# shichaoy/pop_up_slam

Hardware: AMD Instinct MI355X
Metric: graph-solve iters/sec + final chi2, 1k-pose/5k-edge plane graph (higher is better)
Workload: dtype f64; 1 GPU; C2 synthetic corridor: 1000 SE3 poses, 200 planes, 5000 plane edges, 999 odometry edges (BASELINE.json configs[1], seed 42); jacobian_mode=numeric, total_lm_solves=805

## Files before the change

pop_up_slam_amd/csrc/pps_api.cpp:

```cpp
#include "pps_graph.h"

using namespace pps;
using namespace pps_impl;

namespace pps {
Switches read_switches() {
  auto on = [](const char* k) { return getenv(k) != nullptr; };
  auto num = [](const char* k, long long dflt) { const char* e = getenv(k); return e && *e ? atoll(e) : dflt; };
  Switches s;
  s.k1_thread_form = on("PPS_K1_THREAD_FORM");
  {
    long long plain = num("PPS_PLAIN_SCHEDULE", 0);
    if (on("PPS_PLAIN_SCHEDULE") && plain <= 0) plain = 15;
    s.no_preassemble = (plain & 1) != 0; s.no_solve_flow = (plain & 2) != 0; s.no_root_fuse = (plain & 4) != 0; s.split_expand = (plain & 8) != 0;
  }
  s.no_spec_lin = on("PPS_NO_SPEC_LIN");
  s.no_dual = on("PPS_NO_DUAL");
  s.no_strip = on("PPS_NO_STRIP");
  s.no_incremental = on("PPS_NO_INCREMENTAL");
  s.no_incr_compact = on("PPS_NO_INCR_COMPACT");
  s.verify_upload = on("PPS_DEBUG_VERIFY_UPLOAD");
  s.multi_levels = on("PPS_MULTI_LEVELS");
  s.multi_thread_form = on("PPS_MULTI_THREAD_FORM");
  s.debug_drop_flag = (int)num("PPS_DEBUG_DROP_FLAG", 0);
  if (on("PPS_DEBUG_DROP_FLAG") && s.debug_drop_flag < 1) s.debug_drop_flag = 1;
  s.trace = (int)num("PPS_TRACE", 0);
  if (on("PPS_TRACE") && s.trace < 1) s.trace = 1;
  {
    long long tm = num("PPS_TIMING", 0);
    if (on("PPS_TIMING") && tm <= 0) tm = 7;
    s.analysis_timing = (tm & 1) != 0; s.upload_timing = (tm & 2) != 0; s.multi_timing = (tm & 8) ? 2 : ((tm & 4) ? 1 : 0);
  }
  s.multi_split = (int)num("PPS_MULTI_SPLIT", 0);
  s.multi_thread_factors = num("PPS_MULTI_THREAD_FACTORS", 120000);
  return s;
}
}

namespace pps_impl {
void report_front_trace(pps_graph* g) {
  const Analysis& A = g->an;
  std::vector<long long> tr((size_t)A.n_fronts * 8);
  (void)hipMemcpy(tr.data(), g->dev.trace, tr.size() * 8, hipMemcpyDeviceToHost);
  if (g->dev.trace_solve) {
    for (int l = A.n_levels - 1; l >= 0; l--) {
      double ph[5] = {0, 0, 0, 0, 0}, gap = 0; int n = 0, ng = 0;
      for (int s2 = 0; s2 < A.n_fronts; s2++) {
        if (A.f_level[s2] != l) continue;
        n++;
        for (int k = 0; k < 5; k++) ph[k] += (double)(tr[(size_t)s2 * 8 + k + 1] - tr[(size_t)s2 * 8 + k]);
        const int par = A.f_parent[s2];
        if (par >= 0) { gap += (double)(tr[(size_t)s2 * 8] - tr[(size_t)par * 8 + 5]); ng++; }
      }
      if (!n) continue;
      fprintf(stderr, "  solve level %d (%d fronts): panel load %.0f boundary values %.0f y - L_B^T x_b %.0f back-substitution %.0f store %.0f | start after parent's end %.0f\n",
              l, n, ph[0] / n, ph[1] / n, ph[2] / n, ph[3] / n, ph[4] / n, ng ? gap / ng : 0.0);
    }
  } else {
    double acc[5] = {0, 0, 0, 0, 0};
    std::vector<double> lvl_tot(A.n_levels, 0.0); std::vector<int> lvl_n(A.n_levels, 0);
    for (int s2 = 0; s2 < A.n_fronts; s2++) {
      for (int k = 0; k < 5; k++) acc[k] += (double)(tr[(size_t)s2 * 8 + k + 1] - tr[(size_t)s2 * 8 + k]);
      lvl_tot[A.f_level[s2]] += (double)(tr[(size_t)s2 * 8 + 5] - tr[(size_t)s2 * 8]); lvl_n[A.f_level[s2]]++;
    }
    { double pn = 0, tr2 = 0; for (int s2 = 0; s2 < A.n_fronts; s2++) { pn += (double)tr[(size_t)s2 * 8 + 6]; tr2 += (double)tr[(size_t)s2 * 8 + 7]; }
      fprintf(stderr, "PPS_TRACE elimination split: panel %.0f trailing %.0f cycles per front\n", pn / A.n_fronts, tr2 / A.n_fronts); }
    fprintf(stderr, "PPS_TRACE mean cycles per front: zero %.0f gather %.0f extend-add %.0f eliminate %.0f store %.0f\n",
// ... 523 lines not shown
```

pop_up_slam_amd/csrc/pps_device.h:

```cpp
#pragma once

#include <hip/hip_runtime.h>

#include <cstdint>

namespace pps {

struct DevGraph {
  int n_pose = 0, n_plane = 0, pose_ld = 0, plane_ld = 0;
  double *pose_est = nullptr, *pose_lin = nullptr;
  double *plane_est = nullptr, *plane_lin = nullptr;
  int *pose_voff = nullptr, *plane_voff = nullptr;
  int n_obs = 0, n_odo = 0, n_pp = 0, n_lp = 0;
  int obs_ld = 0, odo_ld = 0, pp_ld = 0, lp_ld = 0;
  int *obs_pose = nullptr, *obs_plane = nullptr; double *obs_meas = nullptr, *obs_w = nullptr;
  int n_obs_fixed = 0; double* obs_ray = nullptr;
  int *odo_a = nullptr, *odo_b = nullptr;         double *odo_meas = nullptr, *odo_w = nullptr;
  int *pp_pose = nullptr;                          double *pp_meas = nullptr, *pp_w = nullptr;
  int *lp_plane = nullptr;                         double *lp_meas = nullptr, *lp_w = nullptr;
  double* J = nullptr;
  int64_t joff_obs = 0, joff_odo = 0, joff_pp = 0, joff_lp = 0;
  double* P = nullptr;
  int64_t poff_obs = 0;
  double* H = nullptr;
  double* L = nullptr;
  double* U = nullptr;
  double* delta = nullptr;
  int n_scalars = 0;
  int n_fronts = 0, n_levels = 0, max_front = 0, n_segs = 0, n_blocks = 0;
  int *f_p = nullptr, *f_b = nullptr, *f_poff = nullptr;
  int* pidx = nullptr;
  int64_t *f_Loff = nullptr, *f_Uoff = nullptr;
  int *f_bidx_off = nullptr, *bidx = nullptr;
  int *f_child_off = nullptr, *child = nullptr;
  int *f_cmap_off = nullptr, *cmap = nullptr;
  int *level_fronts = nullptr;
  int *f_asm_off = nullptr, *asm_blk = nullptr, *asm_lrow = nullptr, *asm_lcol = nullptr;
  int *asm_el0 = nullptr, *asm_fsz = nullptr;
  int *blk_rows = nullptr, *blk_cols = nullptr, *blk_size = nullptr, *blk_nseg = nullptr;
  int64_t* blk_hoff = nullptr;
  int *seg_blk = nullptr, *seg_c0 = nullptr, *seg_cnt = nullptr;
  int64_t* seg_hoff = nullptr;
  int* contrib = nullptr;
  int n_mseg = 0; int* mseg_blk = nullptr;
  int *f_el_off = nullptr, *el_src = nullptr, *el_tgt = nullptr;
  int *blk_doff = nullptr, *blk_dst = nullptr;
  double* Hf = nullptr;
  int64_t* f_ea_off = nullptr; int* ea_tgt = nullptr;
  int *grp_lvl_off = nullptr, *glvl_front_off = nullptr, *glvl_fronts = nullptr;
  int* grp_span = nullptr;
  int *frec = nullptr, *crec = nullptr, *srec = nullptr;
  int* obs_dir = nullptr;
  int* k3_flag = nullptr;
  int* nd_segs = nullptr; int n_nd_segs = 0;
  int* k2_single = nullptr; int n_k2_single = 0;
  int* k2_multi = nullptr; int n_k2_multi = 0;
  int* k2_finish = nullptr; int n_k2_finish = 0;
  int* k2t = nullptr; int n_k2t_big = 0, n_k2t_small = 0, n_k2t_spec = 0;
  int *cls_off = nullptr, *cls_fronts = nullptr;
  double* chi2_partials = nullptr;
  int chi2_blocks = 0;
  double* dn_partials = nullptr;
  unsigned int* ticket = nullptr;
  double* result_dev = nullptr;
  long long* trace = nullptr;
  int trace_solve = 0;
  int no_strip = 0;
  unsigned sw = 0;
  double step_ac[4] = {0, 0, 0, 0};
  double* gwork = nullptr;
  int64_t gwork_stride = 0;
};

constexpr double kStatusInternal = 64.0;
enum : unsigned { SW_K1_THREAD_FORM = 1u, SW_NO_SOLVE_FLOW = 2u, SW_NO_ROOT_FUSE = 4u, SW_DEBUG_DROP_FLAG = 8u, SW_DEBUG_DROP_XFLAG = 16u };
struct Switches {
  bool k1_thread_form = false;
  bool no_preassemble = false;
  bool no_solve_flow = false;
  bool no_root_fuse = false;
  bool split_expand = false;
  bool no_spec_lin = false;
  bool no_dual = false;
  bool no_strip = false;
  bool no_incremental = false;
  bool no_incr_compact = false;
  bool verify_upload = false;
  bool multi_levels = false, multi_thread_form = false;
  int debug_drop_flag = 0;
  int trace = 0;
  bool analysis_timing = false, upload_timing = false;
  int multi_timing = 0;
  int multi_split = 0;
  long long multi_thread_factors = 120000;
  unsigned dev_bits() const {
    return (k1_thread_form ? SW_K1_THREAD_FORM : 0u) | (no_solve_flow ? SW_NO_SOLVE_FLOW : 0u) | (no_root_fuse ? SW_NO_ROOT_FUSE : 0u) |
           (debug_drop_flag == 1 ? SW_DEBUG_DROP_FLAG : 0u) | (debug_drop_flag == 2 ? SW_DEBUG_DROP_XFLAG : 0u);
  }
};
Switches read_switches();

struct LinGuard {
  const double* chi[2];
  const double* pose[2];
  const double* plane[2];
  double error;
  int on, single;
  int want = -1;
};

struct SpecLin {
  double *J, *P, *H, *Hf;
  int which;
};

unsigned long long launch_count();
void count_launch();
#define PPS_LAUNCH(...) do { ::pps::count_launch(); hipLaunchKernelGGL(__VA_ARGS__); } while (0)
#define PPS_LAUNCH_EV(ev0, ev1, kernel, grid, block, lds, st, ...)                                                     \
  do {                                                                                                                 \
    ::pps::count_launch();                                                                                             \
    if (ev0) hipExtLaunchKernelGGL(kernel, grid, block, lds, st, ev0, ev1, 0, __VA_ARGS__);                            \
    else hipLaunchKernelGGL(kernel, grid, block, lds, st, __VA_ARGS__);                                                \
  } while (0)

hipError_t step_constants(double ac[4]);
hipError_t launch_linearize(const DevGraph& d, int mode, bool at_estimate, hipStream_t st, const LinGuard* guard = nullptr, hipEvent_t ev0 = nullptr,
                            hipEvent_t ev1 = nullptr);
hipError_t launch_hblocks(const DevGraph& d, hipStream_t st, const LinGuard* guard = nullptr, bool products = true);
bool k1_lane_form(const DevGraph& d, int mode);
bool k1_products(const DevGraph& d, int mode);
hipError_t launch_factor_level(const DevGraph& d, int level_begin, int level_count, int level_max_front, double lambda,
                               hipStream_t st);
hipError_t launch_backsolve_level(const DevGraph& d, int level_begin, int level_count, hipStream_t st);
struct DualAlt {
  double *L, *U, *delta, *result_dev, *chi2_partials, *dn_partials;
  unsigned int* ticket;
  double lambda;
};
hipError_t launch_band_all(const DevGraph& d, const DualAlt* alt, int n_groups, int nwaves_factor, int nwaves_solve, int max_front, int max_panel,
                           int max_group_fronts, double lambda, int epoch, hipStream_t st, hipEvent_t ev0 = nullptr, hipEvent_t ev1 = nullptr);
int band_all_solve_waves(int max_panel, int max_group_fronts);
hipError_t launch_band_factor(const DevGraph& d, int grp_begin, int grp_count, int nwaves, int max_front, double lambda, hipStream_t st,
                              hipEvent_t ev0 = nullptr, hipEvent_t ev1 = nullptr, bool pre = false);
hipError_t launch_band_solve(const DevGraph& d, int grp_begin, int grp_count, int nwaves, int max_panel, int max_group_fronts, hipStream_t st,
                             const DualAlt* alt = nullptr);
hipError_t launch_band_factor_dual(const DevGraph& d, const DualAlt& alt, int grp_begin, int grp_count, int nwaves, int max_front, double lambda,
                                   hipStream_t st, hipEvent_t ev0 = nullptr, hipEvent_t ev1 = nullptr, bool pre = false);
bool band_root_fusable(const DevGraph& d, int grp_count, int max_front);
hipError_t launch_band_root(const DevGraph& d, const DualAlt* alt, int grp, int nwaves_factor, int nwaves_solve, int max_front, int max_panel,
// ... 96 lines not shown
```

pop_up_slam_amd/csrc/pps_front_reg.h:

```cpp
#pragma once
#include <type_traits>

#include "pps_regtile.h"

namespace pps {

#ifndef PPS_TR
#define PPS_TR(k) do { if (d.trace && lane == 0) d.trace[(size_t)s * 8 + (k)] = clock64(); } while (0)
#endif

__device__ __forceinline__ int tri(int i) { return (i * (i + 1)) >> 1; }
__device__ __forceinline__ int tri24(int i) { return __mul24(i, i + 1) >> 1; }

template <int NT, bool TR, bool STRIP, int W = 8, class G>
__device__ __forceinline__ void front_reg_eliminate(const G& d, int rec, double* F, double* P) {
  const int lane = threadIdx.x & 63;
  const int s = __builtin_amdgcn_readlane(rec, 0), p = __builtin_amdgcn_readlane(rec, 1), b = __builtin_amdgcn_readlane(rec, 2);
  const int l16 = lane & 15, lq = lane >> 4;
  const int f = p + b, fa = f + 1;
  const bool strip = STRIP && fa > kRegRows;
  constexpr bool R5 = NT == 5;
  const int mr = STRIP ? fa : f;
  (void)s;
  double4_t c[NT * (NT + 1) / 2];
#pragma unroll
  for (int ti = 0; ti < NT; ti++)
#pragma unroll
    for (int r = 0; r < 4; r++) {
      const int row = 16 * ti + lq + 4 * r;
      const double* Fr = F + (tri24(row < mr ? row : 0) + l16);
#pragma unroll
      for (int tj = 0; tj <= ti; tj++) c[tile_id(ti, tj)][r] = Fr[16 * tj];
    }
  double y = 0.0;
  if (!STRIP) { const double t = F[lane <= f ? tri24(f) + lane : 0]; y = lane < f ? t : 0.0; }
  __builtin_amdgcn_wave_barrier();
  double* __restrict__ Lp = d.L + (((long long)__builtin_amdgcn_readlane(rec, 10) << 32) | (unsigned int)__builtin_amdgcn_readlane(rec, 9));
  long long cyc_panel = 0, cyc_trail = 0;
  bool bad = false;
  auto panel_step = [&](const int K) __attribute__((always_inline)) {
    const long long tk0 = (TR && d.trace) ? clock64() : 0;
    const int nb = p - K < W ? p - K : W;
    const bool two = nb > 4;
    const int tjK = K >> 4, c0 = K & 15;
    switch (tjK) {
      case 0: reg_extract_panel8<0, NT>(c, P, c0, lane); break;
      case 1: reg_extract_panel8<1, NT>(c, P, c0, lane); break;
      case 2: if (NT > 2) reg_extract_panel8<(NT > 2 ? 2 : 1), NT>(c, P, c0, lane); break;
      default: if (NT > 3) reg_extract_panel8<(NT > 3 ? 3 : NT - 1), NT>(c, P, c0, lane); break;
    }
    const int row2 = kRegRows + (lane & 15);
    const bool has2 = STRIP && strip && lane < 16 && row2 < fa;
    if (has2 && !R5) {
#pragma unroll
      for (int m = 0; m < 8; m++) P[row2 * kP8Stride + m] = F[tri(row2) + K + m];
    }
    __builtin_amdgcn_wave_barrier();
    double r[8];
#pragma unroll
    for (int m = 0; m < 8; m++) r[m] = P[lane * kP8Stride + m];
    if (!STRIP) {
#pragma unroll
      for (int m = 0; m < 8; m++) { const double q = readlane_d(y, K + m); r[m] = lane == f ? q : r[m]; }
    }
    const Chol4 c1 = chol4(readlane_d(r[0], K), readlane_d(r[0], K + 1), readlane_d(r[1], K + 1), readlane_d(r[0], K + 2), readlane_d(r[1], K + 2),
                           readlane_d(r[2], K + 2), readlane_d(r[0], K + 3), readlane_d(r[1], K + 3), readlane_d(r[2], K + 3), readlane_d(r[3], K + 3), nb, bad);
    double x[8];
    trsm4(c1, r[0], r[1], r[2], r[3], x[0], x[1], x[2], x[3]);
// ... 51 lines not shown
        if (nb > 5) lrow[5] = yy[5];
        if (nb > 6) lrow[6] = yy[6];
        if (nb > 7) lrow[7] = yy[7];
      }
    }
    __builtin_amdgcn_wave_barrier();
    if (STRIP && strip && !R5) {
      const int cmin = K + nb;
      const bool v0 = lq < nb, v1 = lq + 4 < nb;
      const double a4r = P[(kRegRows + l16) * kP8Stride + lq], a4s = P[(kRegRows + l16) * kP8Stride + 4 + lq];
      const double a40 = v0 ? -a4r : 0.0, a41 = v1 ? -a4s : 0.0;
#pragma unroll 1
      for (int tj = cmin >> 4; tj < 5; tj++) {
        const double br = P[(16 * tj + l16) * kP8Stride + lq], bs = P[(16 * tj + l16) * kP8Stride + 4 + lq];
        const double b0 = v0 ? br : 0.0, b1 = v1 ? bs : 0.0;
        const int col = 16 * tj + l16;
        double4_t t;
        bool ok[4];
#pragma unroll
        for (int q = 0; q < 4; q++) {
          const int row = kRegRows + lq + 4 * q;
          ok[q] = row < fa && col <= row && col >= cmin;
          const double v = F[ok[q] ? tri(row) + col : 0];
          t[q] = ok[q] ? v : 0.0;
        }
        t = __builtin_amdgcn_mfma_f64_16x16x4f64(a40, b0, t, 0, 0, 0);
        if (two) t = __builtin_amdgcn_mfma_f64_16x16x4f64(a41, b1, t, 0, 0, 0);
#pragma unroll
        for (int q = 0; q < 4; q++) {
          const int row = kRegRows + lq + 4 * q;
          if (ok[q]) F[tri(row) + col] = t[q];
        }
      }
    }
    const long long tk1 = (TR && d.trace) ? clock64() : 0;
    switch (tjK) {
      case 0: reg_trailing8<0, NT>(c, P, nb, lane, (K + W) >> 4, c0 + nb < 16); break;
      case 1: reg_trailing8<1, NT>(c, P, nb, lane, (K + W) >> 4, c0 + nb < 16); break;
      case 2: if (NT > 2) reg_trailing8<(NT > 2 ? 2 : 1), NT>(c, P, nb, lane, (K + W) >> 4, c0 + nb < 16); break;
      default: if (NT > 3) reg_trailing8<(NT > 3 ? 3 : NT - 1), NT>(c, P, nb, lane, (K + W) >> 4, c0 + nb < 16); break;
    }
    __builtin_amdgcn_wave_barrier();
    if (TR && d.trace) { const long long tk2 = clock64(); cyc_panel += tk1 - tk0; cyc_trail += tk2 - tk1; }
  };
  if constexpr (NT == 5) {
#pragma clang loop unroll(disable)
    for (int K = 0; K < p; K += W) panel_step(K);
  } else {
    for (int K = 0; K < p; K += W) panel_step(K);
  }
  if (bad && lane == 0) raise_status(&d.result_dev[2], 1.0);
  if (TR) PPS_TR(4);
  if (TR && d.trace && lane == 0) { d.trace[(size_t)s * 8 + 6] = cyc_panel; d.trace[(size_t)s * 8 + 7] = cyc_trail; }
  double* __restrict__ Us = d.U + (((long long)__builtin_amdgcn_readlane(rec, 12) << 32) | (unsigned int)__builtin_amdgcn_readlane(rec, 11));
  const unsigned trash_u = (unsigned)(__mul24(b + 1, b + 1) - 1);
#pragma unroll
  for (int ti = 0; ti < NT; ti++) {
    if (16 * ti >= mr) continue;
    int rbase[4]; bool rok[4];
#pragma unroll
    for (int q = 0; q < 4; q++) { const int row = 16 * ti + lq + 4 * q; rok[q] = row < mr; rbase[q] = tri24(row - p) - p; }
#pragma unroll
    for (int tj = 0; tj <= ti; tj++) {
      if (16 * tj + 15 < p) continue;
      const int col = 16 * tj + l16;
#pragma unroll
      for (int q = 0; q < 4; q++) {
        const int row = 16 * ti + lq + 4 * q;
        const bool ok = rok[q] && col <= row && col >= p;
        Us[ok ? (unsigned)(rbase[q] + col) : trash_u] = c[tile_id(ti, tj)][q];
      }
    }
  }
  if (STRIP && strip && !R5) {
    for (int q = kRegRows; q < fa; q++)
      for (int col = p + lane; col <= q; col += 64) Us[tri(q - p) + col - p] = F[tri(q) + col];
  }
  if (!STRIP) Us[(lane >= p && lane <= f) ? (unsigned)(tri24(b) + lane - p) : trash_u] = lane < f ? y : 0.0;
  if (TR) PPS_TR(5);
}

}
```

pop_up_slam_amd/csrc/pps_k3.hip:

```cpp
#include <algorithm>
#include <atomic>
#include <cstdlib>

#include <hip/hip_ext.h>

#include "pps_kcommon.h"
#include "pps_regtile.h"
#include "pps_front_reg.h"

namespace pps {


constexpr int kLdsLimitBytes = 160 * 1024 - 1024;

int lds_front_limit() {
  int fa = 1;
  while ((size_t)(fa + 1) * ((fa + 1) | 1) * 8 <= (size_t)kLdsLimitBytes) fa++;
  return fa - 1;
}

template <bool USE_LDS>
__global__ __launch_bounds__(256) void k_front_factor(DevGraph d, int level_begin, double lambda) {
  extern __shared__ double lds[];
  const int s = d.level_fronts[level_begin + blockIdx.x];
// ... 380 lines not shown
__device__ __forceinline__ void el_apply(const ElBatch<N>& q, double damp, double* __restrict__ F, int tr) {
  if constexpr (ORIG) {
#pragma unroll
    for (int u = 0; u < N; u++) {
      const int t = q.tg[u] >= 0 ? (q.tg[u] & 0x3fffffff) : tr;
      F[t] = (q.tg[u] & (1 << 30)) && q.tg[u] >= 0 ? q.v[u] * damp : q.v[u];
    }
    return;
  }
  int t[N]; double old[N];
#pragma unroll
  for (int u = 0; u < N; u++) { t[u] = q.tg[u] >= 0 ? q.tg[u] : tr; old[u] = F[t[u]]; }
#pragma unroll
  for (int u = 0; u < N; u++) F[t[u]] = old[u] + q.v[u];
}
template <int NPRE> struct FrontPre { ElBatch<NPRE> q; int crv; };
template <int NPRE>
__device__ __forceinline__ void front_pre_issue(const DevGraph& d, int rec, int lane, FrontPre<NPRE>& o) {
  const int e0 = __builtin_amdgcn_readlane(rec, 3), e1 = __builtin_amdgcn_readlane(rec, 4);
  const int cr0 = __builtin_amdgcn_readlane(rec, 5), nch = __builtin_amdgcn_readlane(rec, 6);
  el_issue(d.el_tgt, d.Hf, e0, e1, lane, o.q);
  o.crv = (lane < 8 * nch) ? d.crec[(size_t)cr0 * 8 + lane] : 0;
}
__device__ __forceinline__ void front_clear(int rec, int lane, double* __restrict__ F) {
  const int ntri = tri(__builtin_amdgcn_readlane(rec, 1) + __builtin_amdgcn_readlane(rec, 2) + 1);
  double2* __restrict__ F2 = reinterpret_cast<double2*>(F);
  const int n2 = ntri >> 1;
#pragma unroll 4
  for (int i = lane; i < n2; i += 64) F2[i] = make_double2(0.0, 0.0);
  if (lane == 0) F[ntri - 1] = 0.0;
  __builtin_amdgcn_wave_barrier();
}
template <int NPRE>
__device__ __forceinline__ void front_pre_finish(const DevGraph& d, int rec, int lane, const FrontPre<NPRE>& o, double damp, double* __restrict__ F, int tr) {
  const int e0 = __builtin_amdgcn_readlane(rec, 3), e1 = __builtin_amdgcn_readlane(rec, 4);
  el_apply<true>(o.q, damp, F, tr);
  for (int e = e0 + 64 * NPRE; e < e1; e += 64 * 8) { ElBatch<8> q; el_issue(d.el_tgt, d.Hf, e, e1, lane, q); __builtin_amdgcn_wave_barrier(); el_apply<true>(q, damp, F, tr); }
  __builtin_amdgcn_wave_barrier();
}
struct XGroup { int* flag; int epoch; };
__device__ __forceinline__ void xg_post(const XGroup& x, int s) {
  __builtin_amdgcn_fence(__ATOMIC_RELEASE, "agent");
  if ((threadIdx.x & 63) == 0) __hip_atomic_store(x.flag + s, x.epoch, __ATOMIC_RELAXED, __HIP_MEMORY_SCOPE_AGENT);
}
__device__ __forceinline__ void xg_wait(const DevGraph& d, const XGroup& x, int s) {
  int spin = 0;
  while (__hip_atomic_load(x.flag + s, __ATOMIC_RELAXED, __HIP_MEMORY_SCOPE_AGENT) != x.epoch) {
    if (++spin >= (1 << 21)) { if ((threadIdx.x & 63) == 0) raise_status(&d.result_dev[2], kStatusInternal); break; }
    __builtin_amdgcn_s_sleep(2);
  }
  __builtin_amdgcn_fence(__ATOMIC_ACQUIRE, "agent");
}
template <bool XG = false>
__device__ __forceinline__ void front_extend_add(const DevGraph& d, int rec, int crv0, int lane, double* __restrict__ F, int tr, const XGroup* xg = nullptr) {
  const int cr0 = __builtin_amdgcn_readlane(rec, 5), nch = __builtin_amdgcn_readlane(rec, 6);
  for (int cb = 0; cb < nch; cb += 8) {
    const int crv = cb == 0 ? crv0 : ((lane < 8 * (nch - cb)) ? d.crec[(size_t)(cr0 + cb) * 8 + lane] : 0);
    auto child = [&](int cj, int& n, const double* __restrict__& Uc, const int* __restrict__& tgc) {
      n = __builtin_amdgcn_readlane(crv, 8 * cj);
      const long long uo = ((long long)__builtin_amdgcn_readlane(crv, 8 * cj + 2) << 32) | (unsigned int)__builtin_amdgcn_readlane(crv, 8 * cj + 1);
      const long long eo = ((long long)__builtin_amdgcn_readlane(crv, 8 * cj + 4) << 32) | (unsigned int)__builtin_amdgcn_readlane(crv, 8 * cj + 3);
      Uc = d.U + uo; tgc = d.ea_tgt + eo;
    };
    int cj = 0;
    for (; cj < 8 && cb + cj < nch; cj++) {
      int n; const double* Uc; const int* tgc;
      child(cj, n, Uc, tgc);
      if (XG) { if (__builtin_amdgcn_readlane(crv, 8 * cj + 6)) xg_wait(d, *xg, __builtin_amdgcn_readlane(crv, 8 * cj + 5)); }
      for (int e = 0; e < n; e += 64 * kEaDepth) { ElBatch<kEaDepth> q; el_issue(tgc, Uc, e, n, lane, q); __builtin_amdgcn_wave_barrier(); el_apply<false>(q, 0.0, F, tr); }
      __builtin_amdgcn_wave_barrier();
    }
  }
}

constexpr int kPanelWBand = 4;
constexpr int kPanelWLevel = 8;
constexpr int kPanelWWide = 8;
template <bool TR>
__device__ __forceinline__ void front_assemble(const DevGraph& d, int rec, double lambda, double* F, int tr) {
  const int lane = threadIdx.x & 63;
  const int s = __builtin_amdgcn_readlane(rec, 0);
  (void)s;
  if (TR) PPS_TR(0);
  FrontPre<8> pre;
  front_pre_issue(d, rec, lane, pre);
  front_clear(rec, lane, F);
  if (TR) PPS_TR(1);
  front_pre_finish(d, rec, lane, pre, 1.0 + lambda, F, tr);
  if (TR) PPS_TR(2);
  front_extend_add(d, rec, pre.crv, lane, F, tr);
  if (TR) PPS_TR(3);
}
template <int NT, bool TR, bool STRIP = false, int W = kPanelWBand>
__device__ __forceinline__ void front_eliminate_out(const DevGraph& d, int rec, double* F, double* P) {
  front_reg_eliminate<NT, TR, STRIP, W>(d, rec, F, P);
}
template <int NT, bool TR, bool STRIP = false, int W = kPanelWBand>
__device__ __forceinline__ void wave_front_factor_reg(const DevGraph& d, int rec, double lambda, double* F, double* P, int tr) {
  front_assemble<TR>(d, rec, lambda, F, tr);
  front_eliminate_out<NT, TR, STRIP, W>(d, rec, F, P);
}

template <int K> __device__ __forceinline__ double row_bcast_d(double v) {
  int lo = __double2loint(v), hi = __double2hiint(v);
  lo = __builtin_amdgcn_update_dpp(0, lo, 0x150 + K, 0xf, 0xf, false);
  hi = __builtin_amdgcn_update_dpp(0, hi, 0x150 + K, 0xf, 0xf, false);
  return __hiloint2double(hi, lo);
}

constexpr double kFlowTimeout = kStatusInternal;
__device__ __forceinline__ void flow_wait(const DevGraph& d, int* flow, int q) {
  int spin = 0;
  while (__hip_atomic_load(flow + q, __ATOMIC_RELAXED, __HIP_MEMORY_SCOPE_WORKGROUP) == 0) {
    if (++spin >= (1 << 22)) { if ((threadIdx.x & 63) == 0) raise_status(&d.result_dev[2], kFlowTimeout); break; }
    __builtin_amdgcn_s_sleep(1);
  }
  __builtin_amdgcn_fence(__ATOMIC_ACQUIRE, "workgroup", "local");
}
__device__ __forceinline__ void flow_post(const DevGraph& d, int* flow, int slot, bool top) {
  __builtin_amdgcn_fence(__ATOMIC_RELEASE, "workgroup", "local");
  if ((threadIdx.x & 63) == 0 && !((d.sw & SW_DEBUG_DROP_FLAG) && top))
    __hip_atomic_store(flow + slot, 1, __ATOMIC_RELAXED, __HIP_MEMORY_SCOPE_WORKGROUP);
}


__device__ __forceinline__ void solve_pivot_scale(double (&lk)[16], double dinv) {
#define PPS_SC(U) lk[U] *= row_bcast_d<U>(dinv);
    PPS_SC(1) PPS_SC(2) PPS_SC(3) PPS_SC(4) PPS_SC(5) PPS_SC(6) PPS_SC(7) PPS_SC(8) PPS_SC(9) PPS_SC(10) PPS_SC(11) PPS_SC(12) PPS_SC(13) PPS_SC(14) PPS_SC(15)
#undef PPS_SC
}
template <bool SCALED = false>
__device__ __forceinline__ void solve_pivot_chain(int p, double (&lk)[16], double dinv, double& tj) {
#ifndef PPS_NO_FMA
#pragma clang fp contract(fast)
#endif
    if (!SCALED) solve_pivot_scale(lk, dinv);
#define PPS_BS(U) case U: tj -= lk[U] * row_bcast_d<U>(tj); [[fallthrough]];
    switch (p < 16 ? p - 1 : 15) {
      PPS_BS(15) PPS_BS(14) PPS_BS(13) PPS_BS(12) PPS_BS(11) PPS_BS(10) PPS_BS(9) PPS_BS(8)
      PPS_BS(7) PPS_BS(6) PPS_BS(5) PPS_BS(4) PPS_BS(3) PPS_BS(2)
      case 1: tj -= lk[1] * row_bcast_d<1>(tj); [[fallthrough]];
      default: break;
    }
#undef PPS_BS
    tj *= dinv;
}

template <bool GROUP = true, bool TR = false, bool XG = false>
// ... 262 lines not shown
      double* const Pn = ALIAS ? F : F + lds_doubles_per_wave - kRegRowsMax * kP8Stride;
      const int tr = ALIAS ? lds_doubles_per_wave - 1 : lds_doubles_per_wave - kRegRowsMax * kP8Stride - 1;
      constexpr int WB = kPanelWBand, WR = kPanelWWide;
      if (REG_ONLY || fa <= kRegRowsMax) {
        if (REG_ONLY) front_assemble<TR>(d, rec, lambda, F, tr);
        else if ((fa <= kRegRowsMax && !d.no_strip) || fa <= kRegRows) front_assemble<true>(d, rec, lambda, F, tr);
      }
      if (REG_ONLY && fa <= 33) front_eliminate_out<2, TR, false, REG_STRIP ? WR : WB>(d, rec, F, Pn);
      else if (REG_ONLY && fa <= 49) front_eliminate_out<3, TR, false, REG_STRIP ? WR : WB>(d, rec, F, Pn);
      else if (REG_ONLY && (!REG_STRIP || fa <= kRegRows)) front_eliminate_out<4, TR, false, REG_STRIP ? WR : WB>(d, rec, F, Pn);
      else if (REG_ONLY && R5) front_eliminate_out<5, false, true, WR>(d, rec, F, Pn);
      else if (fa <= kRegRowsMax && !d.no_strip) front_eliminate_out<4, true, true, WR>(d, rec, F, Pn);
      else if (fa <= kRegRows) front_eliminate_out<4, true, false, WR>(d, rec, F, Pn);
      else wave_front_factor(d, s, lambda, F);
    }
    __syncthreads();
  }
}

template <int NPRE>
__device__ __forceinline__ int front_orig_entries(const DevGraph& d, int rec, int lane, double damp, double* F, int tr) {
  FrontPre<NPRE> pre;
  front_pre_issue(d, rec, lane, pre);
  front_clear(rec, lane, F);
  front_pre_finish(d, rec, lane, pre, damp, F, tr);
  return pre.crv;
}
__device__ __forceinline__ int front_orig_entries_sized(const DevGraph& d, int rec, int lane, double damp, double* F, int tr) {
  const int n_el = __builtin_amdgcn_readlane(rec, 4) - __builtin_amdgcn_readlane(rec, 3);
  if (n_el <= 192) return front_orig_entries<3>(d, rec, lane, damp, F, tr);
  return front_orig_entries<8>(d, rec, lane, damp, F, tr);
}

template <bool XG = false>
__device__ __forceinline__ void body_band_factor_pre(const DevGraph& d, int g, double lambda, int lds_doubles_per_wave, double* __restrict__ lds, const XGroup* xg = nullptr) {
  const int wave = uni(threadIdx.x >> 6), lane = threadIdx.x & 63, nw = uni(blockDim.x >> 6);
  const int4 ga = reinterpret_cast<const int4*>(d.grp_span)[2 * (size_t)g], gb = reinterpret_cast<const int4*>(d.grp_span)[2 * (size_t)g + 1];
  const int nl = uni(ga.z);
  const int o0 = uni(ga.x), o1 = uni(ga.w), o2 = uni(gb.x), o3 = uni(gb.y), o4 = uni(gb.z);
  const int n0 = o1 - o0, n1 = nl > 1 ? o2 - o1 : 0, n2 = nl > 2 ? o3 - o2 : 0, n3 = nl > 3 ? o4 - o3 : 0;
  double* F = lds + (size_t)wave * lds_doubles_per_wave;
  const int tr = lds_doubles_per_wave - 1;
  const bool shape_b = n0 + n1 + n2 + n3 <= nw;
  const int b1 = shape_b ? n0 : 0, b2 = shape_b ? n0 + n1 : n1, b3 = b2 + n2;
  int up_ll = 0, up_rec = 0;
  {
    int up_i = 0;
    if (shape_b && wave >= b1 && wave < b1 + n1) { up_ll = 1; up_i = o1 + wave - b1; }
    else if (wave >= b2 && wave < b2 + n2 && (shape_b || wave >= n1)) { up_ll = 2; up_i = o2 + wave - b2; }
    else if (wave >= b3 && wave < b3 + n3) { up_ll = 3; up_i = o3 + wave - b3; }
    if (up_ll) up_rec = d.frec[(size_t)up_i * 16 + (threadIdx.x & 15)];
  }
  const int pre_at = shape_b ? 0 : 1;
  int crv = 0;
  for (int ll = 0; ll < nl; ll++) {
    const int lb = ll == 0 ? 0 : ll == 1 ? b1 : ll == 2 ? b2 : b3;
    const int cnt = ll == 0 ? n0 : ll == 1 ? n1 : ll == 2 ? n2 : n3;
    const int i0 = ll == 0 ? o0 : ll == 1 ? o1 : ll == 2 ? o2 : o3;
    const bool mine = wave >= lb && wave < lb + cnt;
    const bool mine_up = mine && up_ll == ll && ll > pre_at;
    if (mine) {
      const int rec = (up_ll == ll && ll > 0) ? up_rec : d.frec[(size_t)(i0 + wave - lb) * 16 + (threadIdx.x & 15)];
      const int fa = __builtin_amdgcn_readlane(rec, 1) + __builtin_amdgcn_readlane(rec, 2) + 1;
      if (!mine_up) crv = front_orig_entries_sized(d, rec, lane, 1.0 + lambda, F, tr);
      front_extend_add<XG>(d, rec, crv, lane, F, tr, xg);
      if (fa <= 33) front_eliminate_out<2, false, false, kPanelWBand>(d, rec, F, F);
      else if (fa <= 49) front_eliminate_out<3, false, false, kPanelWBand>(d, rec, F, F);
      else front_eliminate_out<4, false, false, kPanelWBand>(d, rec, F, F);
      if (XG) { if (__builtin_amdgcn_readlane(rec, 13) >= 0 && !(d.sw & SW_DEBUG_DROP_XFLAG)) xg_post(*xg, __builtin_amdgcn_readlane(rec, 0)); }
    } else if (ll == pre_at && up_ll > pre_at) {
      crv = front_orig_entries_sized(d, up_rec, lane, 1.0 + lambda, F, tr);
    }
    __syncthreads();
  }
}

template <bool REG_ONLY>
__global__ __launch_bounds__(512) void k_band_factor(DevGraph d, DualAlt alt, int grp_begin, double lambda, int lds_doubles_per_wave) {
  extern __shared__ double lds[];
  if (blockIdx.y) { d.L = alt.L; d.U = alt.U; d.delta = alt.delta; d.result_dev = alt.result_dev; lambda = alt.lambda; }
  body_band_factor<REG_ONLY>(d, grp_begin + blockIdx.x, lambda, lds_doubles_per_wave, lds);
}

template <bool PRE, bool FLOW>
__global__ __launch_bounds__(512) void k_band_root(DevGraph d, DualAlt alt, int grp, double lambda, int per_wave_factor, int per_wave_solve, int mg) {
  extern __shared__ double lds[];
  if (blockIdx.y) { d.L = alt.L; d.U = alt.U; d.delta = alt.delta; d.result_dev = alt.result_dev; lambda = alt.lambda; }
  if (PRE) body_band_factor_pre(d, grp, lambda, per_wave_factor, lds); else body_band_factor<true>(d, grp, lambda, per_wave_factor, lds);
  if (FLOW) body_band_solve_flow(d, grp, per_wave_solve, lds, mg); else body_band_solve(d, grp, per_wave_solve, lds);
}

__global__ __launch_bounds__(512) void k_band_factor_all(DevGraph d, DualAlt alt, double lambda, int lds_doubles_per_wave, int epoch) {
  extern __shared__ double lds[];
  XGroup xg{d.k3_flag, epoch};
  if (blockIdx.y) { d.L = alt.L; d.U = alt.U; d.delta = alt.delta; d.result_dev = alt.result_dev; lambda = alt.lambda; xg.flag += d.n_fronts; }
  body_band_factor_pre<true>(d, blockIdx.x, lambda, lds_doubles_per_wave, lds, &xg);
}
__global__ __launch_bounds__(768) void k_band_solve_all(DevGraph d, DualAlt alt, int n_groups, int lds_doubles_per_wave, int mg, int epoch) {
  extern __shared__ double lds[];
  XGroup xg{d.k3_flag + 2 * d.n_fronts, epoch};
  if (blockIdx.y) { d.L = alt.L; d.U = alt.U; d.delta = alt.delta; d.result_dev = alt.result_dev; xg.flag += d.n_fronts; }
  body_band_solve_flow<false, true>(d, n_groups - 1 - (int)blockIdx.x, lds_doubles_per_wave, lds, mg, &xg);
}

__global__ __launch_bounds__(512) void k_band_factor_pre(DevGraph d, DualAlt alt, int grp_begin, double lambda, int lds_doubles_per_wave) {
  extern __shared__ double lds[];
  if (blockIdx.y) { d.L = alt.L; d.U = alt.U; d.delta = alt.delta; d.result_dev = alt.result_dev; lambda = alt.lambda; }
  body_band_factor_pre(d, grp_begin + blockIdx.x, lambda, lds_doubles_per_wave, lds);
}

__global__ __launch_bounds__(512) void k_band_factor_lean_trace(DevGraph d, DualAlt alt, int grp_begin, double lambda, int lds_doubles_per_wave) {
  extern __shared__ double lds[];
  body_band_factor<true, false, true>(d, grp_begin + blockIdx.x, lambda, lds_doubles_per_wave, lds);
}

__global__ __launch_bounds__(256) __attribute__((amdgpu_waves_per_eu(1, 1)))
void k_band_factor_r5(DevGraph d, DualAlt alt, int grp_begin, double lambda, int lds_doubles_per_wave) {
  extern __shared__ double lds[];
  if (blockIdx.y) { d.L = alt.L; d.U = alt.U; d.delta = alt.delta; d.result_dev = alt.result_dev; lambda = alt.lambda; }
  body_band_factor<true, true, false, true>(d, grp_begin + blockIdx.x, lambda, lds_doubles_per_wave, lds);
}
// ... 475 lines not shown
```

pop_up_slam_amd/csrc/pps_symbolic.cpp:

```cpp
#include "pps_symbolic.h"

#include <algorithm>
#include <chrono>
#include <cstdio>
#include <cstdlib>
#include <cstring>
#include <cmath>
#include <cstdio>
#include <functional>
#include <numeric>
#include <queue>

namespace pps {
namespace {

struct TNode {
  std::vector<int> piv;
  std::vector<int> kids;
};

struct DissectMemo { int first, last, count, t0, t1; std::vector<int> planes; };

struct Builder {
  const std::vector<SymNode>& nodes;
// ... 1010 lines not shown
    int off = 0;
    for (int k = f_pos0[s]; k < f_pos0[s] + f_npiv[s]; k++) { loc[A.order[k]] = off; off += nodes[A.order[k]].dim; }
    for (int v : bnd[s]) { loc[v] = off; off += nodes[v].dim; }
    const int fsz = A.f_p[s] + A.f_b[s];
    for (int blk : asm_of[s]) {
      const int v = blk_v[blk - B0], u = blk_u[blk - B0];
      if (loc[v] < 0 || loc[u] < 0) { *msg = "internal: H block outside its front"; return 0; }
      A.asm_blk.push_back(blk); A.asm_lrow.push_back(loc[v]); A.asm_lcol.push_back(loc[u]);
      const int rows = A.blk_rows[blk], cols = A.blk_cols[blk];
      const bool diag = v == u;
      A.asm_el0.push_back((int)A.el_total);
      if (blk_is_direct_slot[blk - B0] >= 0) A.obs_dir[3 * (size_t)blk_is_direct_slot[blk - B0] + 1] = (int)A.el_total;
      A.asm_fsz.push_back(fsz);
      A.el_total += diag ? rows * (rows + 1) / 2 + rows : rows * cols;
    }
    A.f_asm_off[s + 1] = (int)A.asm_blk.size();
    A.f_el_off[s + 1] = (int)A.el_total;
    for (int k = f_pos0[s]; k < f_pos0[s] + f_npiv[s]; k++) loc[A.order[k]] = -1;
    for (int v : bnd[s]) loc[v] = -1;
  }
  lap("H blocks / lists");
  {
    A.frec.assign((size_t)F * 16, 0);
    A.crec.clear();
    std::vector<int> pos_of(F, -1);
    for (int i = 0; i < F; i++) pos_of[A.glvl_fronts[i]] = i;
    std::vector<int> grp_first(F, 0);
    for (int g2 = 0; g2 < A.n_groups; g2++) {
      const int i0 = A.glvl_front_off[A.grp_lvl_off[g2]], i1 = A.glvl_front_off[A.grp_lvl_off[g2 + 1]];
      for (int i = i0; i < i1; i++) grp_first[i] = i0;
    }
    for (int i = 0; i < F; i++) {
      const int s2 = A.glvl_fronts[i];
      int* r = &A.frec[(size_t)i * 16];
      r[0] = s2; r[1] = A.f_p[s2]; r[2] = A.f_b[s2]; r[3] = A.f_el_off[s2]; r[4] = A.f_el_off[s2 + 1];
      r[5] = (int)(A.crec.size() / 8); r[6] = A.f_child_off[s2 + 1] - A.f_child_off[s2];
      r[7] = A.f_poff[s2]; r[8] = A.f_bidx_off[s2];
      r[9] = (int)(A.f_Loff[s2] & 0xffffffffLL); r[10] = (int)(A.f_Loff[s2] >> 32);
      r[11] = (int)(A.f_Uoff[s2] & 0xffffffffLL); r[12] = (int)(A.f_Uoff[s2] >> 32);
      r[13] = -1;
      r[14] = -1;
      r[15] = A.f_cmap_off[s2];
      {
        const int par = A.f_parent[s2];
        const int Bn2 = std::max(1, A.band_levels);
        if (par >= 0 && A.f_level[par] / Bn2 == A.f_level[s2] / Bn2) r[14] = pos_of[par] - grp_first[pos_of[par]];
        else if (par >= 0) r[13] = par;
      }
      for (int ci = A.f_child_off[s2]; ci < A.f_child_off[s2 + 1]; ci++) {
        const int c = A.child[ci];
        const int bc1 = A.f_b[c] + 1;
        int cr[8] = {bc1 * (bc1 + 1) / 2, (int)(A.f_Uoff[c] & 0xffffffffLL), (int)(A.f_Uoff[c] >> 32),
                     (int)(A.f_ea_off[c] & 0xffffffffLL), (int)(A.f_ea_off[c] >> 32), c,
                     A.f_level[c] / std::max(1, A.band_levels) != A.f_level[s2] / std::max(1, A.band_levels) ? 1 : 0, 0};
        A.crec.insert(A.crec.end(), cr, cr + 8);
      }
    }
    {
      A.cls_off.assign((size_t)A.n_levels * 3 + 1, 0);
      A.cls_fronts.assign(F, 0);
      std::vector<int> raw((size_t)A.n_levels * 3, 0);
      auto rows_cls = [&](int s2) { const int f = A.f_p[s2] + A.f_b[s2]; return f <= 32 ? 0 : (f <= 48 ? 1 : 2); };
      for (int s2 = 0; s2 < F; s2++) raw[(size_t)A.f_level[s2] * 3 + rows_cls(s2)]++;
      std::vector<signed char> up((size_t)A.n_levels * 3, 0);
      for (int l = 0; l < A.n_levels; l++) {
        int* r = &raw[(size_t)l * 3];
        signed char* u = &up[(size_t)l * 3];
        u[0] = 0; u[1] = 1; u[2] = 2;
        if (r[1] > 0 && r[1] * 16 <= r[2]) { u[1] = 2; r[2] += r[1]; r[1] = 0; }
        if (r[0] > 0) {
          if (r[1] > 0 && r[0] * 16 <= r[1]) u[0] = 1;
          else if (r[1] == 0 && r[2] > 0 && r[0] * 16 <= r[2]) u[0] = 2;
        }
      }
      auto cls_of = [&](int s2) { return (int)up[(size_t)A.f_level[s2] * 3 + rows_cls(s2)]; };
      for (int i = 0; i < F; i++) { const int s2 = A.glvl_fronts[i]; A.cls_off[(size_t)A.f_level[s2] * 3 + cls_of(s2) + 1]++; }
      for (size_t k = 0; k + 1 < A.cls_off.size(); k++) A.cls_off[k + 1] += A.cls_off[k];
      std::vector<int> w(A.cls_off.begin(), A.cls_off.end() - 1);
      for (int i = 0; i < F; i++) { const int s2 = A.glvl_fronts[i]; A.cls_fronts[w[(size_t)A.f_level[s2] * 3 + cls_of(s2)]++] = i; }
    }
    A.srec.resize((size_t)A.n_segs * 8, 0);
    for (int sg = S0; sg < A.n_segs; sg++) {
      const int bk = A.seg_blk[sg];
      int* r = &A.srec[(size_t)sg * 8];
      r[0] = A.blk_rows[bk]; r[1] = A.blk_cols[bk]; r[2] = A.blk_size[bk]; r[3] = A.seg_c0[sg]; r[4] = A.seg_cnt[sg];
      r[5] = (int)A.seg_hoff[sg]; r[6] = A.blk_doff[bk]; r[7] = A.blk_nseg[bk];
    }
    lap("packed records");
  }
  A.kept.fronts = reuse ? F0 : 0; A.kept.fronts_lists = reuse ? F0b : 0; A.kept.blocks = reuse ? B0 : 0; A.kept.segs = reuse ? S0 : 0;
  A.kept.contribs = reuse ? C0 : 0; A.kept.nd_segs = reuse ? nd_kept : 0;
  if (C && !general_ordering) {
    if (reuse && !offsets_changed && C->nodes.size() <= nodes.size() && C->factors.size() <= factors.size()) {
      C->nodes.insert(C->nodes.end(), nodes.begin() + C->nodes.size(), nodes.end());
      C->factors.insert(C->factors.end(), factors.begin() + C->factors.size(), factors.end());
    } else { C->nodes = nodes; C->factors = factors; }
    C->prm = prm;
    C->dense = B.dense;
    C->tree.swap(B.tree);
    C->memo.swap(B.memo);
    C->memo_of_first.assign(N, -1);
    C->memo_next.assign(C->memo.size(), -1);
    for (int mi = (int)C->memo.size() - 1; mi >= 0; mi--) {
      const int fp = C->memo[mi].first;
      if (fp < 0) continue;
      C->memo_next[mi] = C->memo_of_first[fp];
      C->memo_of_first[fp] = mi;
// ... 110 lines not shown
```

Baseline: 17230 LM iters/s.

## Hand child update matrices to parents through LDS within band factor groups

Inside the band-factor kernel, a child front whose parent lives in the same band group now writes its update (Schur complement) matrix into that wave's LDS region instead of global U. The parent's extend-add then reads it back from LDS using a per-child wave index that is now recorded in the child record. This is meant to remove global-memory write and read traffic for intra-group handover. It relies on each wave's LDS slot staying intact until the parent consumes it. The old global path remains available through a new plain-schedule bit.

Measured after the change: 17230 LM iters/s (median of 2 runs). Within noise of the previous version (-0.0%).

```diff
diff --git a/pop_up_slam_amd/csrc/pps_api.cpp b/pop_up_slam_amd/csrc/pps_api.cpp
--- a/pop_up_slam_amd/csrc/pps_api.cpp
+++ b/pop_up_slam_amd/csrc/pps_api.cpp
@@ -11,8 +11,9 @@
   s.k1_thread_form = on("PPS_K1_THREAD_FORM");
   {
     long long plain = num("PPS_PLAIN_SCHEDULE", 0);
-    if (on("PPS_PLAIN_SCHEDULE") && plain <= 0) plain = 15;
+    if (on("PPS_PLAIN_SCHEDULE") && plain <= 0) plain = 31;
     s.no_preassemble = (plain & 1) != 0; s.no_solve_flow = (plain & 2) != 0; s.no_root_fuse = (plain & 4) != 0; s.split_expand = (plain & 8) != 0;
+    s.global_handover = (plain & 16) != 0;
   }
   s.no_spec_lin = on("PPS_NO_SPEC_LIN");
   s.no_dual = on("PPS_NO_DUAL");
diff --git a/pop_up_slam_amd/csrc/pps_device.h b/pop_up_slam_amd/csrc/pps_device.h
--- a/pop_up_slam_amd/csrc/pps_device.h
+++ b/pop_up_slam_amd/csrc/pps_device.h
@@ -73,13 +73,14 @@
 };
 
 constexpr double kStatusInternal = 64.0;
-enum : unsigned { SW_K1_THREAD_FORM = 1u, SW_NO_SOLVE_FLOW = 2u, SW_NO_ROOT_FUSE = 4u, SW_DEBUG_DROP_FLAG = 8u, SW_DEBUG_DROP_XFLAG = 16u };
+enum : unsigned { SW_K1_THREAD_FORM = 1u, SW_NO_SOLVE_FLOW = 2u, SW_NO_ROOT_FUSE = 4u, SW_DEBUG_DROP_FLAG = 8u, SW_DEBUG_DROP_XFLAG = 16u, SW_GLOBAL_HANDOVER = 32u };
 struct Switches {
   bool k1_thread_form = false;
   bool no_preassemble = false;
   bool no_solve_flow = false;
   bool no_root_fuse = false;
   bool split_expand = false;
+  bool global_handover = false;
   bool no_spec_lin = false;
   bool no_dual = false;
   bool no_strip = false;
@@ -95,7 +96,8 @@
   long long multi_thread_factors = 120000;
   unsigned dev_bits() const {
     return (k1_thread_form ? SW_K1_THREAD_FORM : 0u) | (no_solve_flow ? SW_NO_SOLVE_FLOW : 0u) | (no_root_fuse ? SW_NO_ROOT_FUSE : 0u) |
-           (debug_drop_flag == 1 ? SW_DEBUG_DROP_FLAG : 0u) | (debug_drop_flag == 2 ? SW_DEBUG_DROP_XFLAG : 0u);
+           (debug_drop_flag == 1 ? SW_DEBUG_DROP_FLAG : 0u) | (debug_drop_flag == 2 ? SW_DEBUG_DROP_XFLAG : 0u) |
+           (global_handover ? SW_GLOBAL_HANDOVER : 0u);
   }
 };
 Switches read_switches();
diff --git a/pop_up_slam_amd/csrc/pps_front_reg.h b/pop_up_slam_amd/csrc/pps_front_reg.h
--- a/pop_up_slam_amd/csrc/pps_front_reg.h
+++ b/pop_up_slam_amd/csrc/pps_front_reg.h
@@ -12,8 +12,9 @@
 __device__ __forceinline__ int tri(int i) { return (i * (i + 1)) >> 1; }
 __device__ __forceinline__ int tri24(int i) { return __mul24(i, i + 1) >> 1; }
 
-template <int NT, bool TR, bool STRIP, int W = 8, class G>
-__device__ __forceinline__ void front_reg_eliminate(const G& d, int rec, double* F, double* P) {
+template <int NT, bool TR, bool STRIP, int W = 8, bool LDSU = false, class G>
+__device__ __forceinline__ void front_reg_eliminate(const G& d, int rec, double* F, double* P, double* Ul = nullptr, int trl = 0) {
+  static_assert(!(LDSU && STRIP), "the strip rows live in the LDS triangle: their update matrix goes to global memory");
   const int lane = threadIdx.x & 63;
   const int s = __builtin_amdgcn_readlane(rec, 0), p = __builtin_amdgcn_readlane(rec, 1), b = __builtin_amdgcn_readlane(rec, 2);
   const int l16 = lane & 15, lq = lane >> 4;
@@ -171,31 +172,37 @@
   if (bad && lane == 0) raise_status(&d.result_dev[2], 1.0);
   if (TR) PPS_TR(4);
   if (TR && d.trace && lane == 0) { d.trace[(size_t)s * 8 + 6] = cyc_panel; d.trace[(size_t)s * 8 + 7] = cyc_trail; }
-  double* __restrict__ Us = d.U + (((long long)__builtin_amdgcn_readlane(rec, 12) << 32) | (unsigned int)__builtin_amdgcn_readlane(rec, 11));
-  const unsigned trash_u = (unsigned)(__mul24(b + 1, b + 1) - 1);
-#pragma unroll
-  for (int ti = 0; ti < NT; ti++) {
-    if (16 * ti >= mr) continue;
-    int rbase[4]; bool rok[4];
-#pragma unroll
-    for (int q = 0; q < 4; q++) { const int row = 16 * ti + lq + 4 * q; rok[q] = row < mr; rbase[q] = tri24(row - p) - p; }
-#pragma unroll
-    for (int tj = 0; tj <= ti; tj++) {
-      if (16 * tj + 15 < p) continue;
-      const int col = 16 * tj + l16;
-#pragma unroll
-      for (int q = 0; q < 4; q++) {
-        const int row = 16 * ti + lq + 4 * q;
-        const bool ok = rok[q] && col <= row && col >= p;
-        Us[ok ? (unsigned)(rbase[q] + col) : trash_u] = c[tile_id(ti, tj)][q];
-      }
-    }
+  auto store_u = [&](auto* __restrict__ Us, const unsigned trash_u) __attribute__((always_inline)) {
+#pragma unroll
+    for (int ti = 0; ti < NT; ti++) {
+      if (16 * ti >= mr) continue;
+      int rbase[4]; bool rok[4];
+#pragma unroll
+      for (int q = 0; q < 4; q++) { const int row = 16 * ti + lq + 4 * q; rok[q] = row < mr; rbase[q] = tri24(row - p) - p; }
+#pragma unroll
+      for (int tj = 0; tj <= ti; tj++) {
+        if (16 * tj + 15 < p) continue;
+        const int col = 16 * tj + l16;
+#pragma unroll
+        for (int q = 0; q < 4; q++) {
+          const int row = 16 * ti + lq + 4 * q;
+          const bool ok = rok[q] && col <= row && col >= p;
+          Us[ok ? (unsigned)(rbase[q] + col) : trash_u] = c[tile_id(ti, tj)][q];
+        }
+      }
+    }
+    if (STRIP && strip && !R5) {
+      for (int q = kRegRows; q < fa; q++)
+        for (int col = p + lane; col <= q; col += 64) Us[tri(q - p) + col - p] = F[tri(q) + col];
+    }
+    if (!STRIP) Us[(lane >= p && lane <= f) ? (unsigned)(tri24(b) + lane - p) : trash_u] = lane < f ? y : 0.0;
+  };
+  if (LDSU && Ul != nullptr) {
+    __builtin_amdgcn_wave_barrier();
+    store_u(Ul, (unsigned)trl);
+  } else {
+    store_u(d.U + (((long long)__builtin_amdgcn_readlane(rec, 12) << 32) | (unsigned int)__builtin_amdgcn_readlane(rec, 11)), (unsigned)(__mul24(b + 1, b + 1) - 1));
   }
-  if (STRIP && strip && !R5) {
-    for (int q = kRegRows; q < fa; q++)
-      for (int col = p + lane; col <= q; col += 64) Us[tri(q - p) + col - p] = F[tri(q) + col];
-  }
-  if (!STRIP) Us[(lane >= p && lane <= f) ? (unsigned)(tri24(b) + lane - p) : trash_u] = lane < f ? y : 0.0;
   if (TR) PPS_TR(5);
 }
 
diff --git a/pop_up_slam_amd/csrc/pps_k3.hip b/pop_up_slam_amd/csrc/pps_k3.hip
--- a/pop_up_slam_amd/csrc/pps_k3.hip
+++ b/pop_up_slam_amd/csrc/pps_k3.hip
@@ -456,7 +456,8 @@
   __builtin_amdgcn_fence(__ATOMIC_ACQUIRE, "agent");
 }
 template <bool XG = false>
-__device__ __forceinline__ void front_extend_add(const DevGraph& d, int rec, int crv0, int lane, double* __restrict__ F, int tr, const XGroup* xg = nullptr) {
+__device__ __forceinline__ void front_extend_add(const DevGraph& d, int rec, int crv0, int lane, double* __restrict__ F, int tr, const XGroup* xg = nullptr,
+                                                 const double* lds_u = nullptr, int lds_doubles_per_wave = 0) {
   const int cr0 = __builtin_amdgcn_readlane(rec, 5), nch = __builtin_amdgcn_readlane(rec, 6);
   for (int cb = 0; cb < nch; cb += 8) {
     const int crv = cb == 0 ? crv0 : ((lane < 8 * (nch - cb)) ? d.crec[(size_t)(cr0 + cb) * 8 + lane] : 0);
@@ -471,7 +472,12 @@
       int n; const double* Uc; const int* tgc;
       child(cj, n, Uc, tgc);
       if (XG) { if (__builtin_amdgcn_readlane(crv, 8 * cj + 6)) xg_wait(d, *xg, __builtin_amdgcn_readlane(crv, 8 * cj + 5)); }
-      for (int e = 0; e < n; e += 64 * kEaDepth) { ElBatch<kEaDepth> q; el_issue(tgc, Uc, e, n, lane, q); __builtin_amdgcn_wave_barrier(); el_apply<false>(q, 0.0, F, tr); }
+      if (lds_u != nullptr && __builtin_amdgcn_readlane(crv, 8 * cj + 6) == 0) {
+        const double* __restrict__ Ul = lds_u + (size_t)__builtin_amdgcn_readlane(crv, 8 * cj + 7) * lds_doubles_per_wave;
+        for (int e = 0; e < n; e += 64 * kEaDepth) { ElBatch<kEaDepth> q; el_issue(tgc, Ul, e, n, lane, q); __builtin_amdgcn_wave_barrier(); el_apply<false>(q, 0.0, F, tr); }
+      } else {
+        for (int e = 0; e < n; e += 64 * kEaDepth) { ElBatch<kEaDepth> q; el_issue(tgc, Uc, e, n, lane, q); __builtin_amdgcn_wave_barrier(); el_apply<false>(q, 0.0, F, tr); }
+      }
       __builtin_amdgcn_wave_barrier();
     }
   }
@@ -495,9 +501,9 @@
   front_extend_add(d, rec, pre.crv, lane, F, tr);
   if (TR) PPS_TR(3);
 }
-template <int NT, bool TR, bool STRIP = false, int W = kPanelWBand>
-__device__ __forceinline__ void front_eliminate_out(const DevGraph& d, int rec, double* F, double* P) {
-  front_reg_eliminate<NT, TR, STRIP, W>(d, rec, F, P);
+template <int NT, bool TR, bool STRIP = false, int W = kPanelWBand, bool LDSU = false>
+__device__ __forceinline__ void front_eliminate_out(const DevGraph& d, int rec, double* F, double* P, double* Ul = nullptr, int trl = 0) {
+  front_reg_eliminate<NT, TR, STRIP, W, LDSU>(d, rec, F, P, Ul, trl);
 }
 template <int NT, bool TR, bool STRIP = false, int W = kPanelWBand>
 __device__ __forceinline__ void wave_front_factor_reg(const DevGraph& d, int rec, double lambda, double* F, double* P, int tr) {
@@ -866,6 +872,7 @@
     if (up_ll) up_rec = d.frec[(size_t)up_i * 16 + (threadIdx.x & 15)];
   }
   const int pre_at = shape_b ? 0 : 1;
+  const bool lds_ho = shape_b && !(d.sw & SW_GLOBAL_HANDOVER);
   int crv = 0;
   for (int ll = 0; ll < nl; ll++) {
     const int lb = ll == 0 ? 0 : ll == 1 ? b1 : ll == 2 ? b2 : b3;
@@ -877,10 +884,11 @@
       const int rec = (up_ll == ll && ll > 0) ? up_rec : d.frec[(size_t)(i0 + wave - lb) * 16 + (threadIdx.x & 15)];
       const int fa = __builtin_amdgcn_readlane(rec, 1) + __builtin_amdgcn_readlane(rec, 2) + 1;
       if (!mine_up) crv = front_orig_entries_sized(d, rec, lane, 1.0 + lambda, F, tr);
-      front_extend_add<XG>(d, rec, crv, lane, F, tr, xg);
-      if (fa <= 33) front_eliminate_out<2, false, false, kPanelWBand>(d, rec, F, F);
-      else if (fa <= 49) front_eliminate_out<3, false, false, kPanelWBand>(d, rec, F, F);
-      else front_eliminate_out<4, false, false, kPanelWBand>(d, rec, F, F);
+      front_extend_add<XG>(d, rec, crv, lane, F, tr, xg, lds_ho ? lds : nullptr, lds_doubles_per_wave);
+      double* const Ul = lds_ho && __builtin_amdgcn_readlane(rec, 14) >= 0 ? F : nullptr;
+      if (fa <= 33) front_eliminate_out<2, false, false, kPanelWBand, true>(d, rec, F, F, Ul, tr);
+      else if (fa <= 49) front_eliminate_out<3, false, false, kPanelWBand, true>(d, rec, F, F, Ul, tr);
+      else front_eliminate_out<4, false, false, kPanelWBand, true>(d, rec, F, F, Ul, tr);
       if (XG) { if (__builtin_amdgcn_readlane(rec, 13) >= 0 && !(d.sw & SW_DEBUG_DROP_XFLAG)) xg_post(*xg, __builtin_amdgcn_readlane(rec, 0)); }
     } else if (ll == pre_at && up_ll > pre_at) {
       crv = front_orig_entries_sized(d, up_rec, lane, 1.0 + lambda, F, tr);
diff --git a/pop_up_slam_amd/csrc/pps_symbolic.cpp b/pop_up_slam_amd/csrc/pps_symbolic.cpp
--- a/pop_up_slam_amd/csrc/pps_symbolic.cpp
+++ b/pop_up_slam_amd/csrc/pps_symbolic.cpp
@@ -1086,7 +1086,8 @@
         const int bc1 = A.f_b[c] + 1;
         int cr[8] = {bc1 * (bc1 + 1) / 2, (int)(A.f_Uoff[c] & 0xffffffffLL), (int)(A.f_Uoff[c] >> 32),
                      (int)(A.f_ea_off[c] & 0xffffffffLL), (int)(A.f_ea_off[c] >> 32), c,
-                     A.f_level[c] / std::max(1, A.band_levels) != A.f_level[s2] / std::max(1, A.band_levels) ? 1 : 0, 0};
+                     A.f_level[c] / std::max(1, A.band_levels) != A.f_level[s2] / std::max(1, A.band_levels) ? 1 : 0,
+                     pos_of[c] - grp_first[pos_of[c]]};
         A.crec.insert(A.crec.end(), cr, cr + 8);
       }
     }
```
